# Sweetroll97/GaussianProcessPathModelling

Measured on AMD Instinct MI355X. Metric: gp_fit_predict_points_per_sec, higher is better.
Workload: dtype f64; 1 GPU; C3: exact GP fit+predict, N=65536 d=3 rbf float64, M=4096, inputs resident in HBM; N=65536, d=3, M=4096, kernel=rbf, block=2048, parallelism=1 gpu

## Files before the change

### gaussianprocesspathmodelling_amd/csrc/gpx_tile.h

```cpp
#pragma once
#include <hip/hip_runtime.h>
#include <stdint.h>

#include "gpx_internal.h"

namespace gpx {
namespace {

template <typename T>
struct Num;
template <>
struct Num<double> {
  typedef double v4 __attribute__((ext_vector_type(4)));
  typedef double slot __attribute__((ext_vector_type(2)));
  static constexpr int SLOT = 2;
  static constexpr int BK = 16;
  static constexpr int KS64 = 4;
  static __device__ __forceinline__ v4 mfma(double a, double b, v4 c) {
    return __builtin_amdgcn_mfma_f64_16x16x4f64(a, b, c, 0, 0, 0);
  }
  static __device__ __forceinline__ int drow(int l4, int r) { return l4 + 4 * r; }
  static __device__ __forceinline__ double rsq(double x) { return rsqrt(x); }
};
template <>
struct Num<float> {
  typedef float v4 __attribute__((ext_vector_type(4)));
  typedef float slot __attribute__((ext_vector_type(4)));
  static constexpr int SLOT = 4;
  static constexpr int BK = 32;
  static constexpr int KS64 = 2;
  static __device__ __forceinline__ v4 mfma(float a, float b, v4 c) {
    return __builtin_amdgcn_mfma_f32_16x16x4f32(a, b, c, 0, 0, 0);
  }
  static __device__ __forceinline__ int drow(int l4, int r) { return 4 * l4 + r; }
  static __device__ __forceinline__ float rsq(float x) { return rsqrtf(x); }
};

__device__ __forceinline__ int swz(int row) {
  const int t = ((row >> 1) + 2) & 7;
  return ((t & 3) << 1) | (t >> 2);
}

template <typename T, int BM, int BN, int KSUB = 1>
struct TileShapeG {
  static constexpr int BK = Num<T>::BK;
  static constexpr int A_STAGE = BM * BK * KSUB, B_STAGE = BN * BK * KSUB;
  static constexpr int SMEM_ELEMS = 2 * (A_STAGE + B_STAGE);
};

#define GPX_GLDS16(gptr, lptr)                                                             \
  __builtin_amdgcn_global_load_lds((const __attribute__((address_space(1))) void*)(gptr),  \
                                   (__attribute__((address_space(3))) void*)(lptr), 16, 0, 0)

template <typename T, int BM, int BN, int WVM = 2, int KSUB = 1>
__device__ __forceinline__ void gemm_tile_g(const T* A, int64_t lda, const T* B, int64_t ldb, int K,
                                            typename Num<T>::v4 (&acc)[BM / (16 * WVM)][BN / 32], T* smem) {
  using S = TileShapeG<T, BM, BN, KSUB>;
  using slot_t = typename Num<T>::slot;
  constexpr int BK = S::BK, SL = Num<T>::SLOT;
  constexpr int MT = BM / (16 * WVM), NT = BN / 32, WM = BM / WVM, WN = BN / 2;
  constexpr int IA = BM / (16 * WVM), IB = BN / (16 * WVM);
  constexpr int RQ = 8 * BK;
  const int tid = threadIdx.x;
  const int lane = tid & 63;
  const int wave = __builtin_amdgcn_readfirstlane(tid >> 6);
  const int wr = wave >> 1, wc = wave & 1;
  const int l15 = lane & 15, l4 = lane >> 4;
  T* As = smem;
  T* Bs = smem + 2 * S::A_STAGE;

  const int drow = lane >> 3, dslot = lane & 7;
  const T* ga[IA];
  const T* gb[IB];
#pragma unroll
  for (int q = 0; q < IA; ++q) {
    const int row = (wave * IA + q) * 8 + drow;
    ga[q] = A + (int64_t)row * lda + (dslot ^ swz(row)) * SL;
  }
#pragma unroll
  for (int q = 0; q < IB; ++q) {
    const int row = (wave * IB + q) * 8 + drow;
    gb[q] = B + (int64_t)row * ldb + (dslot ^ swz(row)) * SL;
  }
  T* const la = As + wave * IA * RQ;
  T* const lb = Bs + wave * IB * RQ;

  const int sw = swz(l15);
  const int a_off0 = (wr * WM + l15) * BK + ((2 * l4) ^ sw) * SL;
  const int a_off1 = (wr * WM + l15) * BK + ((2 * l4 + 1) ^ sw) * SL;
  const int b_off0 = (wc * WN + l15) * BK + ((2 * l4) ^ sw) * SL;
  const int b_off1 = (wc * WN + l15) * BK + ((2 * l4 + 1) ^ sw) * SL;

#pragma unroll
  for (int u = 0; u < KSUB; ++u) {
#pragma unroll
    for (int q = 0; q < IA; ++q) GPX_GLDS16(ga[q] + u * BK, la + u * BM * BK + q * RQ);
#pragma unroll
    for (int q = 0; q < IB; ++q) GPX_GLDS16(gb[q] + u * BK, lb + u * BN * BK + q * RQ);
  }
  __syncthreads();

  constexpr int HALF = SL * MT * NT;
  const int KT = K / (BK * KSUB);
  for (int kt = 0; kt < KT; ++kt) {
    const int buf = kt & 1;
    const int64_t ko = (int64_t)(kt + 1 < KT ? kt + 1 : kt) * (BK * KSUB);
#pragma unroll
    for (int u = 0; u < KSUB; ++u) {
      const T* Ab = As + buf * S::A_STAGE + u * BM * BK;
      const T* Bb = Bs + buf * S::B_STAGE + u * BN * BK;
      slot_t a0[MT], b0[NT], a1[MT], b1[NT];
#pragma unroll
      for (int m = 0; m < MT; ++m) a0[m] = *reinterpret_cast<const slot_t*>(Ab + a_off0 + m * 16 * BK);
#pragma unroll
      for (int n = 0; n < NT; ++n) b0[n] = *reinterpret_cast<const slot_t*>(Bb + b_off0 + n * 16 * BK);
#pragma unroll
      for (int m = 0; m < MT; ++m) a1[m] = *reinterpret_cast<const slot_t*>(Ab + a_off1 + m * 16 * BK);
#pragma unroll
      for (int n = 0; n < NT; ++n) b1[n] = *reinterpret_cast<const slot_t*>(Bb + b_off1 + n * 16 * BK);
      {
#pragma unroll
        for (int q = 0; q < IA; ++q)
          GPX_GLDS16(ga[q] + ko + u * BK, la + (buf ^ 1) * S::A_STAGE + u * BM * BK + q * RQ);
#pragma unroll
        for (int q = 0; q < IB; ++q)
          GPX_GLDS16(gb[q] + ko + u * BK, lb + (buf ^ 1) * S::B_STAGE + u * BN * BK + q * RQ);
      }
#pragma unroll
      for (int s = 0; s < SL; ++s)
#pragma unroll
        for (int m = 0; m < MT; ++m)
#pragma unroll
          for (int n = 0; n < NT; ++n) acc[m][n] = Num<T>::mfma(a0[m][s], b0[n][s], acc[m][n]);
#pragma unroll
      for (int s = 0; s < SL; ++s)
#pragma unroll
        for (int m = 0; m < MT; ++m)
#pragma unroll
          for (int n = 0; n < NT; ++n) acc[m][n] = Num<T>::mfma(a1[m][s], b1[n][s], acc[m][n]);
      __builtin_amdgcn_sched_group_barrier(0x100, MT + NT, 0);
#pragma unroll
      for (int i = 0; i < MT + NT; ++i) {
        __builtin_amdgcn_sched_group_barrier(0x8, HALF / (2 * (MT + NT)), 0);
        __builtin_amdgcn_sched_group_barrier(0x100, 1, 0);
      }
#pragma unroll
      for (int i = 0; i < IA + IB; ++i) {
        __builtin_amdgcn_sched_group_barrier(0x8, HALF / (2 * (IA + IB)), 0);
        __builtin_amdgcn_sched_group_barrier(0x20, 1, 0);
      }
      if (KSUB > 1) __builtin_amdgcn_sched_group_barrier(0x8, HALF, 0);
    }
    __builtin_amdgcn_sched_barrier(0);
    __syncthreads();
  }
}

template <typename V4, int MT, int NT>
__device__ __forceinline__ void zero_acc(V4 (&acc)[MT][NT]) {
#pragma unroll
  for (int m = 0; m < MT; ++m)
#pragma unroll
    for (int n = 0; n < NT; ++n) acc[m][n] = (V4){0, 0, 0, 0};
}

template <typename T, int BM, int BN, int MODE, int WVM = 2>
__device__ __forceinline__ void store_tile(T* C, int64_t ldc,
                                           const typename Num<T>::v4 (&acc)[BM / (16 * WVM)][BN / 32]) {
  constexpr int NT = BN / 32;
  const int lane = threadIdx.x & 63;
  const int wave = threadIdx.x >> 6;
  const int wr = wave >> 1, wc = wave & 1;
  const int l4 = lane >> 4;
  T* Cw = C + (int64_t)(wr * (BM / WVM)) * ldc + wc * (BN / 2) + (lane & 15);
#pragma unroll
  for (int m = 0; m < BM / (16 * WVM); ++m) {
    T* Cm = Cw + (int64_t)(m * 16) * ldc;
#pragma unroll
    for (int n = 0; n < NT; ++n)
#pragma unroll
      for (int r = 0; r < 4; ++r) {
        T* dst = &Cm[(int64_t)Num<T>::drow(l4, r) * ldc + n * 16];
        if (MODE == 0)
          unsafeAtomicAdd(dst, -acc[m][n][r]);
        else
          *dst = acc[m][n][r];
      }
  }
}

__host__ __device__ __forceinline__ int64_t xcd_chunk_id(int64_t bid, int64_t nblk) {
  const int64_t q = nblk >> 3, r = nblk & 7, x = bid & 7;
  return (x < r ? x * (q + 1) : r * (q + 1) + (x - r) * q) + (bid >> 3);
}

__host__ __device__ __forceinline__ void tri_coords(int64_t t, int& ti, int& tj) {
  int64_t i = (int64_t)((sqrtf(8.0f * (float)t + 1.0f) - 1.0f) * 0.5f);
  if (i < 0) i = 0;
  while (i * (i + 1) / 2 > t) --i;
  while ((i + 1) * (i + 2) / 2 <= t) ++i;
  ti = (int)i;
  tj = (int)(t - i * (i + 1) / 2);
}

template <bool TRI>
__host__ __device__ __forceinline__ bool tile_coords(int64_t lin, int tiles_m, int tiles_n, int sh,
                                            int mask_lower, const BcMask& bc, int& ti, int& tj) {
  const int64_t st = lin >> 6;
  const int inner = (int)(lin & 63);
  if (TRI) {
    const int S = (tiles_m + 7) >> 3;
    const int64_t full = (int64_t)S * (S - 1) / 2 * 64;
    if (lin < full) {
      int i, j;
      tri_coords(st, i, j);
      ti = (i + 1) * 8 + (inner >> 3);
      tj = j * 8 + (inner & 7);
    } else {
      const int64_t id2 = lin - full;
      const int k = (int)(id2 / 36), e = (int)(id2 - (int64_t)k * 36);
      int r = (int)((__builtin_sqrtf(8.0f * (float)e + 1.0f) - 1.0f) * 0.5f);
      if (r * (r + 1) / 2 > e) --r;
      if ((r + 1) * (r + 2) / 2 <= e) ++r;
      ti = k * 8 + r;
      tj = k * 8 + (e - r * (r + 1) / 2);
    }
    return ti < tiles_m && tj < tiles_n;
  } else {
    const int sw = 64 / sh;
    const int sn = (tiles_n + sw - 1) / sw;
    const int sr = (int)(st / sn), sc = (int)(st - (int64_t)sr * sn);
    ti = sr * sh + inner / sw;
    tj = sc * sw + inner % sw;
    if (ti >= tiles_m || tj >= tiles_n) return false;
    if (mask_lower == 1) return tj <= ti;
    if (mask_lower == 2) return tj <= bc.row_tile(ti);
    return true;
  }
}
}
}
```

Measured before the change: 43960 points/s.

## Software-pipeline GEMM tile k-loop with carried MFMA slice and scalar base addressing

Restructures the double-buffered f64 MFMA GEMM inner loop. The last MFMA slice of each k-step is deferred into the next step so it overlaps the next step's LDS reads and the barrier. The loop is unrolled by two with compile-time buffer indices, and each second-half fragment read is interleaved with one async global-to-LDS copy. Global addressing uses a wave-uniform scalar base plus 32-bit per-lane offsets, which cuts VGPR and 64-bit address arithmetic. Risks are 32-bit offset overflow for large lda and heavier reliance on the hand-tuned scheduling barriers.

```diff
diff --git a/gaussianprocesspathmodelling_amd/csrc/gpx_tile.h b/gaussianprocesspathmodelling_amd/csrc/gpx_tile.h
--- a/gaussianprocesspathmodelling_amd/csrc/gpx_tile.h
+++ b/gaussianprocesspathmodelling_amd/csrc/gpx_tile.h
@@ -1,6 +1,8 @@
 #pragma once
 #include <hip/hip_runtime.h>
 #include <stdint.h>
+
+#include <type_traits>
 
 #include "gpx_internal.h"
 
@@ -51,6 +53,13 @@
 #define GPX_GLDS16(gptr, lptr)                                                             \
   __builtin_amdgcn_global_load_lds((const __attribute__((address_space(1))) void*)(gptr),  \
                                    (__attribute__((address_space(3))) void*)(lptr), 16, 0, 0)
+
+template <typename P>
+__device__ __forceinline__ const P* uniform_ptr(const P* p) {
+  const uint64_t v = (uint64_t)p;
+  const uint32_t lo = __builtin_amdgcn_readfirstlane((uint32_t)v), hi = __builtin_amdgcn_readfirstlane((uint32_t)(v >> 32));
+  return (const P*)(((uint64_t)hi << 32) | lo);
+}
 
 template <typename T, int BM, int BN, int WVM = 2, int KSUB = 1>
 __device__ __forceinline__ void gemm_tile_g(const T* A, int64_t lda, const T* B, int64_t ldb, int K,
@@ -70,18 +79,19 @@
   T* Bs = smem + 2 * S::A_STAGE;
 
   const int drow = lane >> 3, dslot = lane & 7;
-  const T* ga[IA];
-  const T* gb[IB];
+  uint32_t oa[IA], ob[IB];
 #pragma unroll
   for (int q = 0; q < IA; ++q) {
     const int row = (wave * IA + q) * 8 + drow;
-    ga[q] = A + (int64_t)row * lda + (dslot ^ swz(row)) * SL;
+    oa[q] = ((uint32_t)(q * 8 + drow) * (uint32_t)lda + (uint32_t)((dslot ^ swz(row)) * SL)) * (uint32_t)sizeof(T);
   }
 #pragma unroll
   for (int q = 0; q < IB; ++q) {
     const int row = (wave * IB + q) * 8 + drow;
-    gb[q] = B + (int64_t)row * ldb + (dslot ^ swz(row)) * SL;
-  }
+    ob[q] = ((uint32_t)(q * 8 + drow) * (uint32_t)ldb + (uint32_t)((dslot ^ swz(row)) * SL)) * (uint32_t)sizeof(T);
+  }
+  const char* const gA = (const char*)uniform_ptr(A + (int64_t)(wave * IA * 8) * lda);
+  const char* const gB = (const char*)uniform_ptr(B + (int64_t)(wave * IB * 8) * ldb);
   T* const la = As + wave * IA * RQ;
   T* const lb = Bs + wave * IB * RQ;
 
@@ -91,40 +101,69 @@
   const int b_off0 = (wc * WN + l15) * BK + ((2 * l4) ^ sw) * SL;
   const int b_off1 = (wc * WN + l15) * BK + ((2 * l4 + 1) ^ sw) * SL;
 
-#pragma unroll
-  for (int u = 0; u < KSUB; ++u) {
-#pragma unroll
-    for (int q = 0; q < IA; ++q) GPX_GLDS16(ga[q] + u * BK, la + u * BM * BK + q * RQ);
-#pragma unroll
-    for (int q = 0; q < IB; ++q) GPX_GLDS16(gb[q] + u * BK, lb + u * BN * BK + q * RQ);
-  }
-  __syncthreads();
+  auto dma = [&](int buf, int kt) __attribute__((always_inline)) {
+    const int64_t kb = (int64_t)kt * (BK * KSUB) * (int64_t)sizeof(T);
+#pragma unroll
+    for (int u = 0; u < KSUB; ++u) {
+#pragma unroll
+      for (int q = 0; q < IA; ++q)
+        GPX_GLDS16(gA + kb + u * BK * (int)sizeof(T) + oa[q], la + buf * S::A_STAGE + u * BM * BK + q * RQ);
+#pragma unroll
+      for (int q = 0; q < IB; ++q)
+        GPX_GLDS16(gB + kb + u * BK * (int)sizeof(T) + ob[q], lb + buf * S::B_STAGE + u * BN * BK + q * RQ);
+    }
+  };
+  slot_t a0[MT], b0[NT], a1[MT], b1[NT];
+  auto carried = [&]() __attribute__((always_inline)) {
+#pragma unroll
+    for (int m = 0; m < MT; ++m)
+#pragma unroll
+      for (int n = 0; n < NT; ++n) acc[m][n] = Num<T>::mfma(a1[m][SL - 1], b1[n][SL - 1], acc[m][n]);
+  };
 
   constexpr int HALF = SL * MT * NT;
+  constexpr int G_RD = HALF / (2 * (MT + NT));
+  constexpr int REST = 2 * HALF - (MT + NT) * G_RD;
   const int KT = K / (BK * KSUB);
-  for (int kt = 0; kt < KT; ++kt) {
-    const int buf = kt & 1;
-    const int64_t ko = (int64_t)(kt + 1 < KT ? kt + 1 : kt) * (BK * KSUB);
+  auto kstep = [&](auto carry_c, auto buf_c, int kt) __attribute__((always_inline)) {
+    constexpr bool CARRY = decltype(carry_c)::value;
+    constexpr int BUF = decltype(buf_c)::value;
+    const int kn = kt + 1 < KT ? kt + 1 : kt;
 #pragma unroll
     for (int u = 0; u < KSUB; ++u) {
-      const T* Ab = As + buf * S::A_STAGE + u * BM * BK;
-      const T* Bb = Bs + buf * S::B_STAGE + u * BN * BK;
-      slot_t a0[MT], b0[NT], a1[MT], b1[NT];
+      const T* Ab = As + BUF * S::A_STAGE + u * BM * BK;
+      const T* Bb = Bs + BUF * S::B_STAGE + u * BN * BK;
+      const bool carry_in = CARRY && u == 0, carry_out = u == KSUB - 1;
 #pragma unroll
       for (int m = 0; m < MT; ++m) a0[m] = *reinterpret_cast<const slot_t*>(Ab + a_off0 + m * 16 * BK);
 #pragma unroll
       for (int n = 0; n < NT; ++n) b0[n] = *reinterpret_cast<const slot_t*>(Bb + b_off0 + n * 16 * BK);
-#pragma unroll
-      for (int m = 0; m < MT; ++m) a1[m] = *reinterpret_cast<const slot_t*>(Ab + a_off1 + m * 16 * BK);
-#pragma unroll
-      for (int n = 0; n < NT; ++n) b1[n] = *reinterpret_cast<const slot_t*>(Bb + b_off1 + n * 16 * BK);
-      {
-#pragma unroll
-        for (int q = 0; q < IA; ++q)
-          GPX_GLDS16(ga[q] + ko + u * BK, la + (buf ^ 1) * S::A_STAGE + u * BM * BK + q * RQ);
-#pragma unroll
-        for (int q = 0; q < IB; ++q)
-          GPX_GLDS16(gb[q] + ko + u * BK, lb + (buf ^ 1) * S::B_STAGE + u * BN * BK + q * RQ);
+      if (carry_in) carried();
+      const int64_t kb = ((int64_t)kn * (BK * KSUB) + u * BK) * (int64_t)sizeof(T);
+      const char* pa = gA + kb;
+      const char* pb = gB + kb;
+      asm("" : "+s"(pa), "+s"(pb));
+      auto read2 = [&](int i) __attribute__((always_inline)) {
+        if (i < MT)
+          a1[i] = *reinterpret_cast<const slot_t*>(Ab + a_off1 + i * 16 * BK);
+        else
+          b1[i - MT] = *reinterpret_cast<const slot_t*>(Bb + b_off1 + (i - MT) * 16 * BK);
+      };
+      auto dma1 = [&](int i) __attribute__((always_inline)) {
+        if (i < IA) {
+          asm("" : "+v"(oa[i]) : "s"(pa));
+          GPX_GLDS16(pa + oa[i], la + (BUF ^ 1) * S::A_STAGE + u * BM * BK + i * RQ);
+        } else {
+          const int q = i - IA;
+          asm("" : "+v"(ob[q]) : "s"(pb));
+          GPX_GLDS16(pb + ob[q], lb + (BUF ^ 1) * S::B_STAGE + u * BN * BK + q * RQ);
+        }
+      };
+      static_assert(MT + NT == IA + IB, "one DMA per second-half fragment read");
+#pragma unroll
+      for (int i = 0; i < MT + NT; ++i) {
+        read2(i);
+        dma1(i);
       }
 #pragma unroll
       for (int s = 0; s < SL; ++s)
@@ -133,27 +172,41 @@
 #pragma unroll
           for (int n = 0; n < NT; ++n) acc[m][n] = Num<T>::mfma(a0[m][s], b0[n][s], acc[m][n]);
 #pragma unroll
-      for (int s = 0; s < SL; ++s)
+      for (int s = 0; s < (carry_out ? SL - 1 : SL); ++s)
 #pragma unroll
         for (int m = 0; m < MT; ++m)
 #pragma unroll
           for (int n = 0; n < NT; ++n) acc[m][n] = Num<T>::mfma(a1[m][s], b1[n][s], acc[m][n]);
       __builtin_amdgcn_sched_group_barrier(0x100, MT + NT, 0);
+      if (carry_in) __builtin_amdgcn_sched_group_barrier(0x8, MT * NT, 0);
 #pragma unroll
       for (int i = 0; i < MT + NT; ++i) {
-        __builtin_amdgcn_sched_group_barrier(0x8, HALF / (2 * (MT + NT)), 0);
+        __builtin_amdgcn_sched_group_barrier(0x8, G_RD, 0);
         __builtin_amdgcn_sched_group_barrier(0x100, 1, 0);
-      }
-#pragma unroll
-      for (int i = 0; i < IA + IB; ++i) {
-        __builtin_amdgcn_sched_group_barrier(0x8, HALF / (2 * (IA + IB)), 0);
         __builtin_amdgcn_sched_group_barrier(0x20, 1, 0);
       }
-      if (KSUB > 1) __builtin_amdgcn_sched_group_barrier(0x8, HALF, 0);
+      if (KSUB > 1) {
+        if (carry_out)
+          __builtin_amdgcn_sched_group_barrier(0x8, REST - MT * NT, 0);
+        else
+          __builtin_amdgcn_sched_group_barrier(0x8, REST, 0);
+      }
     }
     __builtin_amdgcn_sched_barrier(0);
     __syncthreads();
-  }
+  };
+  using std::integral_constant;
+  dma(0, 0);
+  __syncthreads();
+  if (KT < 1) return;
+  kstep(integral_constant<bool, false>{}, integral_constant<int, 0>{}, 0);
+  int kt = 1;
+  for (; kt + 1 < KT; kt += 2) {
+    kstep(integral_constant<bool, true>{}, integral_constant<int, 1>{}, kt);
+    kstep(integral_constant<bool, true>{}, integral_constant<int, 0>{}, kt + 1);
+  }
+  if (kt < KT) kstep(integral_constant<bool, true>{}, integral_constant<int, 1>{}, kt);
+  carried();
 }
 
 template <typename V4, int MT, int NT>
```

Measured after the change: 45100 points/s, median of 6. 1.03x the previous value.
